# Krabbens/edge-diffusion-tts

Hardware: AMD Instinct MI355X
Metric: mel-frames/sec (whole node), 4-step DDIM, hidden=160 L=4, B=256 T=512 (higher is better)
Workload: dtype f32

## Files before the change

### edge-diffusion-tts_amd/csrc/edtts_device.h

```cpp
#pragma once
#include <hip/hip_runtime.h>
#include <stdint.h>
#include <type_traits>

#if !defined(EDTTS_EXPERIMENTS) &&                                                                                                  \
    (defined(EDTTS_STAMPS) || defined(EDTTS_STAMP_HEAD) || defined(EDTTS_STAMP_THREAD) || defined(EDTTS_WAVELOG) ||                 \
     defined(EDTTS_DS_STAMPS) || defined(EDTTS_FAST_BUILD))
#error "diagnostic and build switches are scratch-only: add -DEDTTS_EXPERIMENTS"
#endif
#if defined(EDTTS_W2) || defined(EDTTS_KV2) || defined(EDTTS_SPLITLOAD) || defined(EDTTS_SPLIT_ON) || defined(EDTTS_HANDOVER) ||    \
    defined(EDTTS_H_DMA) || defined(EDTTS_TAIL_RING2) || defined(EDTTS_DS_BURST) || defined(EDTTS_PIN_MASK) ||                      \
    defined(EDTTS_WMAX) || defined(EDTTS_RB) || defined(EDTTS_ABLATE_QKVSTORES) || defined(EDTTS_ABLATE_KVLOADS) ||                 \
    defined(EDTTS_DS_ABL) || defined(EDTTS_DIAG) || defined(EDTTS16_HP) || defined(EDTTS16_KVDEPTH) ||                              \
    defined(EDTTS16_MFMA_SUM) || defined(EDTTS16_EVEN_STEPS) || defined(EDTTS16_QLDS) || defined(EDTTS16_IMG) ||                    \
    defined(EDTTS16_W1) || defined(EDTTS16_NF) || defined(EDTTS16_ABLATE_BARRIER) || defined(EDTTS16_ABLATE_DMA) ||                 \
    defined(EDTTS16_PHASES)
#error "this switch is retired, see DESIGN.md: its variant was decided and the code removed (last present in c6f336d)"
#endif

constexpr int kPinMask = 0x4;
#define EDTTS_PIN_ACC(x) asm volatile("" : "+a"(x))
typedef float f4 __attribute__((ext_vector_type(4)));
typedef float f2 __attribute__((ext_vector_type(2)));

#define EDTTS_MFMA(a, b, c) __builtin_amdgcn_mfma_f32_16x16x4f32((a), (b), (c), 0, 0, 0)
#define EDTTS_DEV __device__ __forceinline__

#ifdef EDTTS_STAMPS
#define STAMP_SEL_HEAD(sel) ((sel) & 0xff)
#define STAMPX(p, i, sel) do { if ((p) && (int)blockIdx.x == ((sel) >> 16) && (int)threadIdx.x == 64 * (((sel) >> 8) & 0xff)) (p)[i] = __builtin_amdgcn_s_memtime(); } while (0)
#else
#define STAMPX(p, i, sel) do { } while (0)
#endif

namespace edtts {

constexpr int kCtxWaves = 4;

template <int H_, int HEADS_, int MEL_, int NF_ = 2>
struct Cfg {
  static constexpr int H = H_, HEADS = HEADS_, MEL = MEL_, NF = NF_;
  static constexpr int WF = 16 * NF;
  static constexpr int QT = NF >= 2 ? 2 : 1;
  static constexpr int NHALF = NF / QT;
  static constexpr int DH = H / HEADS;
  static constexpr int DFULL = DH / 16;
  static constexpr int DREM = DH % 16;
  static constexpr int DT = (DH + 15) / 16;
  static constexpr int DHP = DT * 16;
  static constexpr int HT = H / 16;
  static constexpr int MT = MEL / 16;
  static constexpr int R = H / 2, RT = R / 16;
  static constexpr int VR = (HEADS - 1) * DH + DHP;
  static constexpr int WMAX = 2;
  static constexpr int WAVES0 = (HT * NF * 4 <= 160) ? 4 : 2;
  static constexpr int WAVES = NF == 1 ? 1 : (WAVES0 < WMAX ? WAVES0 : WMAX);
// ... 572 lines not shown
#ifdef EDTTS_STAMPS
        if (hd == STAMP_SEL_HEAD(stamp_sel)) STAMPX(stamps, sidx++, stamp_sel);
#endif
      };
      const int cd = q.cdiag;
      auto chunk_of = [&](int st) { return st >= nchunk ? nchunk - 1 : (st == 0 ? cd : (st <= cd ? st - 1 : st)); };
      constexpr bool HANDOVER = NHALF == 1;
      const bool more = HANDOVER && hd + hstep < C::HEADS;
      auto req_head = [&](int st) { return (more && st == nchunk - 1) ? hd + hstep : hd; };
      auto req_chunk = [&](int st) { return (more && st == nchunk - 1) ? cd : chunk_of(st + 1); };
      step(No{}, cd, req_chunk(0), KA, VA, req_head(0));
      for (int st = 1; st < nchunk; ++st) step(Yes{}, chunk_of(st), req_chunk(st), KA, VA, req_head(st));
#pragma unroll
      for (int ft = 0; ft < QT; ++ft) {
        const float lt = group_sum(hsum(lvec[ft]));
        const float inv = lt > 0.f ? 1.0f / lt : 0.f;
#pragma unroll
        for (int dt = 0; dt < DT; ++dt) O[dt][QT * hf + ft] *= inv;
      }
    }
#ifdef EDTTS_STAMPS
    if (hd == STAMP_SEL_HEAD(stamp_sel)) STAMPX(stamps, sidx++, stamp_sel);
#endif
    if (hd + hstep < C::HEADS) {
      if constexpr (NHALF == 1) {
        load_q(hd + hstep, 0);
        __builtin_amdgcn_sched_barrier(0);
      } else {
        prefetch(geo[0], hd + hstep, 0);
      }
    }
    if constexpr (OMODE == O_LDS) {
      char* ob = obuf + hd * C::OHEAD_BYTES;
#pragma unroll
      for (int dt = 0; dt < DT; ++dt)
#pragma unroll
        for (int ft = 0; ft < NF; ++ft) {
          if (DREM && dt == DT - 1) reinterpret_cast<f2*>(ob + DFULL * NF * 1024 + ft * 512)[lane] = f2{O[dt][ft][0], O[dt][ft][1]};
          else reinterpret_cast<f4*>(ob + (dt * NF + ft) * 1024)[lane] = O[dt][ft];
        }
    } else {
#pragma unroll
      for (int dt = 0; dt < DT; ++dt) {
        if (DREM && dt == DT - 1) ktile_phase<C::HT, WStream<C>::RN_, NF, 2>(ring, O[dt], h);
        else ktile_phase<C::HT>(ring, O[dt], h);
      }
    }
#ifdef EDTTS_STAMPS
    if (hd == STAMP_SEL_HEAD(stamp_sel)) STAMPX(stamps, sidx++, stamp_sel);
#endif
  }
}

EDTTS_DEV void ddim_elem(float x, float e, float s1m, float sab, float sabp, float cdir, float& x0, float& xp) {
#pragma clang fp contract(off)
  float t1 = s1m * e;
  float t2 = x - t1;
  float v = div_rn(t2, sab);
  v = fminf(fmaxf(v, -3.0f), 3.0f);
  x0 = v;
  float t3 = sabp * v;
  float t4 = cdir * e;
  xp = t3 + t4;
}
struct DdimCoef {
  float s1m, sab, sabp, cdir, sigma;
};
EDTTS_DEV DdimCoef ddim_coef(float ab, float abp, float eta) {
#pragma clang fp contract(off)
  DdimCoef c;
  c.s1m = sqrt_rn(1.0f - ab);
  c.sab = sqrt_rn(ab);
  float r1 = div_rn(1.0f - abp, 1.0f - ab);
  float r2 = 1.0f - div_rn(ab, abp);
  float pr = r1 * r2;
  c.sigma = eta * sqrt_rn(pr);
  float s2 = c.sigma * c.sigma;
  float in = 1.0f - abp;
  in = in - s2;
  c.cdir = sqrt_rn(in);
  c.sabp = sqrt_rn(abp);
  return c;
}
EDTTS_DEV float add_mul_rn(float p, float s, float n) {
#pragma clang fp contract(off)
  float t = s * n;
  return p + t;
}

struct DdpmCoef {
  float coef1, coef2, sd;
};
EDTTS_DEV DdpmCoef ddpm_coef(float al, float ab, float be, float var, bool nonzero) {
#pragma clang fp contract(off)
  DdpmCoef c;
  c.coef1 = div_rn(1.0f, sqrt_rn(al));
  float om = 1.0f - ab;
  c.coef2 = div_rn(be, sqrt_rn(om));
  c.sd = (nonzero ? 1.0f : 0.0f) * sqrt_rn(var);
  return c;
}
EDTTS_DEV float ddpm_elem(float x, float e, float n, DdpmCoef c) {
#pragma clang fp contract(off)
  float t1 = c.coef2 * e;
  float t2 = x - t1;
  float mean = c.coef1 * t2;
  float t3 = c.sd * n;
  return mean + t3;
}

struct LmsCoef {
  int mode;
  float p0, p1, c0, c1, rinv, cB, cC;
};
EDTTS_DEV void lms_elem(float x, float out, float h_new, float h_old, const LmsCoef& k, float& x0, float& xn) {
#pragma clang fp contract(off)
// ... 139 lines not shown
```

### edge-diffusion-tts_amd/csrc/edtts_generic.h

```cpp
namespace edtts_gen {

enum { EPI_BIAS = 0, EPI_PE = 1, EPI_RESID = 2, EPI_SWIGLU = 3 };

struct GemmArgs {
  const float* X;
  const float* W;
  const float* bias;
  float* Y;
  const float* pe;
  int M, N, K, ldx, ldy, T;
  int vec_x, vec_w, vec_y;
  DropArgs dr;
};
constexpr int kGBM = 64, kGBN = 64, kGBK = 16, kGLd = kGBK + 1;

template <int EPI, bool DROP = false>
__global__ __launch_bounds__(256) void k_gen_gemm(GemmArgs a) {
  __shared__ float xs[kGBM][kGLd];
  __shared__ float ws[kGBN][kGLd];
  const int tid = threadIdx.x, lane = tid & 63, w = tid >> 6, fq = lane & 15, g = lane >> 4;
  const int m0 = blockIdx.x * kGBM;
  const int n0 = blockIdx.y * (EPI == EPI_SWIGLU ? kGBN / 2 : kGBN);
  const int lr = tid >> 2, lk = 4 * (tid & 3);
  int wrow;
// ... 280 lines not shown
                                                   int H, int n_tok, unsigned* err, const int64_t* s_len) {
  const size_t n = (size_t)rows * H;
  for (size_t i = (size_t)blockIdx.x * blockDim.x + threadIdx.x; i < n; i += (size_t)gridDim.x * blockDim.x) {
    const size_t row = i / H;
    const int c = (int)(i - row * H);
    long tk = (s_len && (int)(row % S) >= utt_len_lane(s_len, (int)(row / S), S)) ? 0 : (long)sem_idx[row];
    if (tk < 0 || tk >= n_tok) {
      if (c == 0) atomicOr(err, (unsigned)EDTTS_IDX_SEM);
      tk = tk < 0 ? 0 : n_tok - 1;
    }
    ctx[i] = tok[(size_t)tk * H + c] + cpe[(size_t)(row % S) * H + c];
  }
}

template <int TAIL>
EDTTS_DEV void tail_elem(const KArgs& a, size_t idx, float e) {
  if (TAIL == TAIL_LMS) {
    const float hn = a.lms.mode >= 2 ? a.h_new[idx] : 0.f, ho = a.lms.mode >= 3 ? a.h_old[idx] : 0.f;
    float v0, vn;
    lms_elem(a.x[idx], e, hn, ho, a.lms, v0, vn);
    a.x0_hist[idx] = v0;
    if (a.x0_all) a.x0_all[idx] = v0;
    a.x_prev[idx] = vn;
  } else if (TAIL == TAIL_VLMS) {
    const float v = a.v_uncond ? cfg_combine(e, a.v_uncond[idx], a.vp.cfg) : e;
    const float hn = a.lms.mode >= 2 ? a.h_new[idx] : 0.f, ho = a.lms.mode >= 3 ? a.h_old[idx] : 0.f;
    float v0, vn;
    lms_elem(a.x[idx], v, hn, ho, a.lms, v0, vn);
    a.x0_hist[idx] = v0;
    if (a.x0_all) a.x0_all[idx] = v0;
    if (a.known != nullptr) {
      const size_t row = (size_t)a.T * a.inj_mel, b = idx / row, r = idx - b * row, per = (size_t)a.inj_frames * a.inj_mel;
      if (r < per) {
        const size_t ki = b * per + r;
        vn = a.known[ki];
        if (a.p_coef2 != 0.f) {
          const float nz = a.noise ? a.noise[ki]
                                   : (a.seeds ? philox_normal4(a.seeds[b], a.step, r >> 2)[(int)(r & 3)] : philox_normal4(a.seed, a.step, ki >> 2)[(int)(ki & 3)]);
          vn = qsample_elem(vn, a.p_coef1, nz, a.p_coef2);
        }
      }
    }
    a.x_prev[idx] = vn;
  } else if (TAIL == TAIL_VPRED) {
    const float v = a.v_uncond ? cfg_combine(e, a.v_uncond[idx], a.vp.cfg) : e;
    a.x_prev[idx] = vpred_elem(a.x[idx], v, a.vp);
  } else if (TAIL == TAIL_DDPM) {
    const unsigned long long ge = a.philox_base + idx;
    const float nz = a.noise ? a.noise[idx] : philox_normal4(a.seed, a.step, ge >> 2)[(int)(ge & 3)];
    const DdpmCoef cf{a.p_coef1, a.p_coef2, a.p_sd};
    a.x_prev[idx] = ddpm_elem(a.x[idx], e, nz, cf);
  } else {
    float v0, vp;
    ddim_elem(a.x[idx], e, a.c_s1m, a.c_sab, a.c_sabp, a.c_dir, v0, vp);
    a.x0[idx] = v0;
    a.x_prev[idx] = vp;
  }
}
template <int TAIL>
EDTTS_DEV void tail_zero_elem(const KArgs& a, size_t idx) {
  if (TAIL == TAIL_LMS || TAIL == TAIL_VLMS) {
    a.x0_hist[idx] = 0.f;
    if (a.x0_all) a.x0_all[idx] = 0.f;
  } else if (TAIL == TAIL_DDIM) {
    a.x0[idx] = 0.f;
  }
  a.x_prev[idx] = 0.f;
}
EDTTS_DEV bool past_len(const int64_t* t_len, bool dbl, size_t idx, int T, int MEL) {
  if (t_len == nullptr) return false;
  const size_t row = idx / MEL;
  return (int)(row % T) >= utt_len_lane(t_len, (int)(row / T), T, dbl);
}
template <int TAIL>
__global__ __launch_bounds__(256) void k_gen_tail(KArgs a, const float* eps, size_t n, int vec, int MEL) {
  const size_t stride = (size_t)gridDim.x * blockDim.x;
  if (vec) {
    for (size_t i = (size_t)blockIdx.x * blockDim.x + threadIdx.x; i < n / 4; i += stride) {
      if constexpr (TAIL == TAIL_VLMS) {
        const size_t row = 4 * i / MEL;
        const int f = (int)(row % a.T);
        const int Tb = a.t_len ? utt_len_of(a.t_len[row / a.T], a.T, a.t_dbl) : a.T;
        tail_store<TAIL>(a, f, Tb, 4 * i, ldg4(eps + 4 * i));
        continue;
      }
      if (past_len(a.t_len, a.t_dbl, 4 * i, a.T, MEL)) tail_zero<TAIL>(a, 4 * i);
      else tail_apply<TAIL>(a, 4 * i, ldg4(eps + 4 * i));
    }
  } else {
    for (size_t i = (size_t)blockIdx.x * blockDim.x + threadIdx.x; i < n; i += stride) {
      if (past_len(a.t_len, a.t_dbl, i, a.T, MEL)) tail_zero_elem<TAIL>(a, i);
      else tail_elem<TAIL>(a, i, eps[i]);
    }
  }
}
__global__ __launch_bounds__(256) void k_gen_zero_past(float* y, const int64_t* t_len, int dbl, size_t n, int T, int MEL) {
  for (size_t i = (size_t)blockIdx.x * blockDim.x + threadIdx.x; i < n; i += (size_t)gridDim.x * blockDim.x)
    if (past_len(t_len, dbl, i, T, MEL)) y[i] = 0.f;
}

}

enum { DROP_ATTN = 0, DROP_CROSS = 1, DROP_ACT = 2, DROP_DOWN = 3 };
struct DropState {
  unsigned k0, k1, thr;
  float scale;
  DropArgs site(int layer, int site_id) const { return DropArgs{k0, k1, 0x30000u + 4u * (unsigned)layer + (unsigned)site_id, thr, scale}; }
};

struct FwdLayerBufs {
  float *crp, *crn, *kv;
  float *qkv, *att1, *lse1;
  float *qc, *att2, *lse2;
  float* act;
  float *h0, *h1, *h2;
};
struct FwdBufs {
  float* ctx;
// ... 201 lines not shown
```

### edge-diffusion-tts_amd/csrc/edtts_kernels.hip

```cpp
#include <hip/hip_runtime.h>
#include <math.h>
#include <stdarg.h>
#include <stdlib.h>
#include <stdio.h>
#include <string.h>
#include <atomic>
#include <initializer_list>
#include <mutex>
#include <vector>

#include "../../include/edtts.h"
#include "edtts_device.h"

using namespace edtts;

static thread_local char g_err[512] = "";
static int fail(int code, const char* fmt, ...) __attribute__((format(printf, 2, 3)));
static int fail(int code, const char* fmt, ...) {
  va_list ap;
  va_start(ap, fmt);
  vsnprintf(g_err, sizeof(g_err), fmt, ap);
  va_end(ap);
  return code;
}
// ... 374 lines not shown
    sidx = a.use_host ? (long)a.step_host[row] : (long)a.step_idx[row];
    if (sidx < 0 || sidx >= a.n_step) {
      if (tid == 0) atomicOr(a.err, (unsigned)EDTTS_IDX_STEP);
      sidx = sidx < 0 ? 0 : a.n_step - 1;
    }
  }
  for (int n = tid; n < H; n += blockDim.x) {
    float acc = a.t3b[n];
#pragma unroll 8
    for (int k = 0; k < H; ++k) acc = fmaf(u[k], a.t3T[(size_t)k * H + n], acc);
    if (sidx >= 0) acc += a.step[(size_t)sidx * H + n];
    a.tcond[(size_t)row * H + n] = acc;
  }
}
__global__ __launch_bounds__(256) void k_cond_ada(CondArgs a) {
  extern __shared__ float sm[];
  const int row = blockIdx.x, lw = blockIdx.y, l = lw >> 1, which = lw & 1, H = a.H;
  for (int k = threadIdx.x; k < H; k += blockDim.x) sm[k] = a.tcond[(size_t)row * H + k];
  __syncthreads();
  const float* WT = a.blob + (which ? a.ada3T[l] : a.ada1T[l]);
  const float* bb = a.blob + (which ? a.ada3b[l] : a.ada1b[l]);
  float* out = a.cond + (((size_t)row * a.L + l) * 2 + which) * 2 * H;
  for (int n = blockIdx.z * blockDim.x + threadIdx.x; n < 2 * H; n += gridDim.z * blockDim.x) {
    float acc = bb[n];
#pragma unroll 8
    for (int k = 0; k < H; ++k) acc = fmaf(sm[k], WT[(size_t)k * 2 * H + n], acc);
    out[n] = n < H ? 1.0f + acc : acc;
  }
}

struct KArgs {
  int B, T, Tp, S, Sp, window, max_pos, max_cpos, n_tok, SD, L;
  const float* x;
  float* h;
  const float *q, *k, *vT;
  float *q_out, *k_out, *vT_out;
  float *kc, *vcT;
  const float* known;
  const unsigned long long* seeds;
  int inj_frames, inj_mel;
  const int64_t* sem_idx;
  const float* sem_feat;
  const float* cond;
  int cond_bstride;
  int layer;
  int ffn_tiles;
  int diag_skip;
  unsigned long long* stamps;
  const float *tok, *semp, *semp_b, *cpe, *inp, *inp_b, *pe;
  const float *n1w, *proj_b, *n2w, *n3w, *up_b, *down_b, *fnw, *fnb, *outp_b;
  const float* stream;
  float *eps, *x_prev, *x0;
  float c_s1m, c_sab, c_sabp, c_dir;
  float p_coef1, p_coef2, p_sd;
  const float* noise;
  unsigned long long seed;
  unsigned long long philox_base;
  unsigned step;
  LmsCoef lms;
  VpredCoef vp;
  const float* v_uncond;
  const float *h_new, *h_old;
  float *x0_hist, *x0_all;
  const int64_t *t_len, *s_len;
  int t_dbl;
};

EDTTS_DEV int utt_len_of(int64_t v, int full, bool dbl) {
  const int hi = dbl ? full >> 1 : full;
  const int n = v < 1 ? 1 : (v > hi ? hi : (int)v);
  return dbl ? 2 * n : n;
}
EDTTS_DEV int utt_len(const int64_t* len, int b, int full, bool dbl = false) {
  if (len == nullptr) return full;
  return utt_len_of(len[__builtin_amdgcn_readfirstlane(b)], full, dbl);
}
EDTTS_DEV int utt_len_lane(const int64_t* len, int b, int full, bool dbl = false) {
  return len == nullptr ? full : utt_len_of(len[b], full, dbl);
}
EDTTS_DEV int live_end(int n) { return (n + 31) & ~31; }

EDTTS_DEV int remap_block(int bid, int nblk) {
  const int q = nblk >> 3, r = nblk & 7, xcd = bid & 7, idx = bid >> 3;
  const int base = xcd < r ? xcd * (q + 1) : r * (q + 1) + (xcd - r) * q;
  return base + idx;
}

struct TileId {
  int b, m0;
  bool valid;
};
EDTTS_DEV TileId wave_tile(int B, int Tp, int waves_per_block, int wave_frames) {
  const int wave = __builtin_amdgcn_readfirstlane(threadIdx.x >> 6);
  const int tpu = Tp / wave_frames;
  int w = remap_block(blockIdx.x, gridDim.x) * waves_per_block + wave;
  TileId t;
  t.valid = w < B * tpu;
  w = t.valid ? w : B * tpu - 1;
  t.b = w / tpu;
  t.m0 = (w - t.b * tpu) * wave_frames;
  return t;
}

template <class C>
EDTTS_DEV void qkv_tail(WStream<C>& ring0, const f4 (&hn)[C::HT][C::NF], const KArgs& a, int b, int m0, int lane) {
  constexpr int NF = C::NF;
// ... 59 lines not shown
  }
  f4 h[C::HT][NF];
#pragma unroll
  for (int nt = 0; nt < C::HT; ++nt) {
    const f4 bias = ldg4(a.inp_b + 16 * nt + 4 * g);
#pragma unroll
    for (int ft = 0; ft < NF; ++ft) h[nt][ft] = bias;
  }
  {
    constexpr int N = C::HT * C::MT;
    static_assert(N % WStream<C>::RN_ == 0 && C::HT % 2 == 0, "in_proj must be a whole number of ring turns");
#pragma unroll
    for (int nt = 0; nt < C::HT; nt += 2)
#pragma unroll
      for (int kt = 0; kt < C::MT; ++kt) {
        const int i = nt * C::MT + 2 * kt;
        const f4& fa = ring.at(i);
        const f4& fb = ring.at(i + 1);
#pragma unroll
        for (int r = 0; r < 4; ++r) {
#pragma unroll
          for (int ft = 0; ft < NF; ++ft) h[nt][ft] = EDTTS_MFMA(fa[r], xin[kt][ft][r], h[nt][ft]);
#pragma unroll
          for (int ft = 0; ft < NF; ++ft) h[nt + 1][ft] = EDTTS_MFMA(fb[r], xin[kt][ft][r], h[nt + 1][ft]);
        }
        ring.template refill_after<N>(i);
        ring.template refill_after<N>(i + 1);
      }
    ring.advance(N);
  }
#pragma unroll
  for (int ft = 0; ft < NF; ++ft) {
    int f = m0 + 16 * ft + fq;
    f = f < a.max_pos ? f : a.max_pos - 1;
#pragma unroll
    for (int nt = 0; nt < C::HT; ++nt) h[nt][ft] += ldg4(a.pe + (size_t)f * C::H + 16 * nt + 4 * g);
  }
  {
    float* hp = a.h + ((size_t)b * a.Tp + m0 + fq) * C::H + 4 * g;
#pragma unroll
    for (int nt = 0; nt < C::HT; ++nt)
#pragma unroll
      for (int ft = 0; ft < NF; ++ft) stg4(hp + 16 * nt + (size_t)ft * 16 * C::H, h[nt][ft]);
  }
  f4 hn[C::HT][NF];
  const float* mod = a.cond + (size_t)b * a.cond_bstride;
  rms_norm_tile<C::HT, NF>(h, a.n1w, mod, g, hn);
  qkv_tail<C>(ring, hn, a, b, m0, lane);
}

enum { TAIL_QKV = 0, TAIL_EPS = 1, TAIL_DDIM = 2, TAIL_DDPM = 3, TAIL_LMS = 4, TAIL_VPRED = 5, TAIL_VLMS = 6 };

template <int TAIL>
EDTTS_DEV void tail_apply(const KArgs& a, size_t idx, f4 ev, bool blend = false) {
  if (TAIL == TAIL_EPS) {
    stg4(a.eps + idx, ev);
  } else if (TAIL == TAIL_LMS) {
    const f4 xv = ldg4(a.x + idx);
    f4 hn = splat(0.f), ho = splat(0.f);
    if (a.lms.mode >= 2) hn = ldg4(a.h_new + idx);
    if (a.lms.mode >= 3) ho = ldg4(a.h_old + idx);
    f4 x0, xn;
#pragma unroll
    for (int r = 0; r < 4; ++r) {
      float v0, vn;
      lms_elem(xv[r], ev[r], hn[r], ho[r], a.lms, v0, vn);
      x0[r] = v0;
      xn[r] = vn;
    }
    stg4(a.x0_hist + idx, x0);
    if (a.x0_all) stg4(a.x0_all + idx, x0);
    stg4(a.x_prev + idx, xn);
  } else if (TAIL == TAIL_VLMS) {
    const bool guided = a.v_uncond != nullptr;
    const f4 xv = ldg4(a.x + idx);
    const f4 vu = ldg4((guided ? a.v_uncond : a.x) + idx);
    f4 hn = splat(0.f), ho = splat(0.f);
    if (a.lms.mode >= 2) hn = ldg4(a.h_new + idx);
    if (a.lms.mode >= 3) ho = ldg4(a.h_old + idx);
    f4 x0, xn;
#pragma unroll
    for (int r = 0; r < 4; ++r) {
      const float v = guided ? cfg_combine(ev[r], vu[r], a.vp.cfg) : ev[r];
      float v0, vn;
      lms_elem(xv[r], v, hn[r], ho[r], a.lms, v0, vn);
      x0[r] = v0;
      xn[r] = vn;
    }
    stg4(a.x0_hist + idx, x0);
    if (a.x0_all) stg4(a.x0_all + idx, x0);
    if (!blend) stg4(a.x_prev + idx, xn);
  } else if (TAIL == TAIL_VPRED) {
    const bool guided = a.v_uncond != nullptr;
    const f4 xv = ldg4(a.x + idx);
    const f4 vu = ldg4((guided ? a.v_uncond : a.x) + idx);
    f4 v, xn;
#pragma unroll
    for (int r = 0; r < 4; ++r) v[r] = guided ? cfg_combine(ev[r], vu[r], a.vp.cfg) : ev[r];
#pragma unroll
    for (int r = 0; r < 4; ++r) xn[r] = vpred_elem(xv[r], v[r], a.vp);
    stg4(a.x_prev + idx, xn);
  } else if (TAIL == TAIL_DDPM) {
    const f4 xv = ldg4(a.x + idx);
    const f4 nz = a.noise ? ldg4(a.noise + idx) : philox_normal4(a.seed, a.step, (a.philox_base + idx) >> 2);
    const DdpmCoef cf{a.p_coef1, a.p_coef2, a.p_sd};
    f4 xp;
#pragma unroll
    for (int r = 0; r < 4; ++r) xp[r] = ddpm_elem(xv[r], ev[r], nz[r], cf);
    stg4(a.x_prev + idx, xp);
  } else {
    const f4 xv = ldg4(a.x + idx);
    f4 x0, xp;
#pragma unroll
    for (int r = 0; r < 4; ++r) {
      float v0, vp;
      ddim_elem(xv[r], ev[r], a.c_s1m, a.c_sab, a.c_sabp, a.c_dir, v0, vp);
      x0[r] = v0;
      xp[r] = vp;
    }
    stg4(a.x0 + idx, x0);
    stg4(a.x_prev + idx, xp);
  }
}
template <int TAIL>
EDTTS_DEV void tail_zero(const KArgs& a, size_t idx) {
  const f4 z = splat(0.f);
  if (TAIL == TAIL_EPS) {
    stg4(a.eps + idx, z);
  } else if (TAIL == TAIL_LMS || TAIL == TAIL_VLMS) {
    stg4(a.x0_hist + idx, z);
    if (a.x0_all) stg4(a.x0_all + idx, z);
    stg4(a.x_prev + idx, z);
  } else if (TAIL == TAIL_DDIM) {
    stg4(a.x0 + idx, z);
    stg4(a.x_prev + idx, z);
  } else {
    stg4(a.x_prev + idx, z);
  }
}
EDTTS_DEV void vlms_blend(const KArgs& a, size_t idx) {
  const size_t row = (size_t)a.T * a.inj_mel, b = idx / row, r = idx - b * row;
  const size_t ki = b * ((size_t)a.inj_frames * a.inj_mel) + r;
  const f4 kv = ldg4(a.known + ki);
  f4 o = kv;
  if (a.p_coef2 != 0.f) {
    const unsigned long long sd = a.seeds ? a.seeds[b] : a.seed;
    const f4 nz = a.noise ? ldg4(a.noise + ki) : philox_normal4(sd, a.step, (a.seeds ? r : ki) >> 2);
#pragma unroll
    for (int e = 0; e < 4; ++e) o[e] = qsample_elem(kv[e], a.p_coef1, nz[e], a.p_coef2);
  }
  stg4(a.x_prev + idx, o);
}
template <int TAIL>
EDTTS_DEV void tail_store(const KArgs& a, int f, int Tb, size_t idx, f4 ev) {
  if constexpr (TAIL == TAIL_VLMS) {
    const bool blend = a.known != nullptr && f < Tb && f < a.inj_frames;
    if (f < Tb) tail_apply<TAIL>(a, idx, ev, blend);
    else tail_zero<TAIL>(a, idx);
    if (blend) vlms_blend(a, idx);
  } else {
    if (f < Tb) tail_apply<TAIL>(a, idx, ev);
    else tail_zero<TAIL>(a, idx);
  }
}

struct QGlobal {
  __amdgpu_buffer_rsrc_t rs;
  unsigned v4, v2;
  int H;
  EDTTS_DEV QGlobal(const float* row_m0, int H_, int fq, int g) : rs(make_rsrc(row_m0)), v4((unsigned)(fq * H_ + 4 * g) * 4u), v2((unsigned)(fq * H_ + 2 * g) * 4u), H(H_) {}
  EDTTS_DEV f4 q4(int ft, int col) const { return bufld4(rs, v4, (unsigned)(ft * 16 * H + col) * 4u); }
  EDTTS_DEV f2 q2(int ft, int col) const { return bufld2(rs, v2, (unsigned)(ft * 16 * H + col) * 4u); }
};
struct QLds {
  const float* b4;
  const float* b2;
  int ld;
  EDTTS_DEV QLds(const float* tile, int ld_, int fq, int g) : b4(tile + fq * ld_ + 4 * g), b2(tile + fq * ld_ + 2 * g), ld(ld_) {}
  EDTTS_DEV f4 q4(int ft, int col) const { return *reinterpret_cast<const f4*>(b4 + ft * 16 * ld + col); }
  EDTTS_DEV f2 q2(int ft, int col) const { return *reinterpret_cast<const f2*>(b2 + ft * 16 * ld + col); }
};

template <class C, int TAIL>
EDTTS_DEV void layer_tile(const KArgs& a, float* smem, int wave, int lane, int b, int m0, int Tb, int Sb) {
  constexpr int NF = C::NF;
  const int fq = lane & 15, g = lane >> 4;
  f4* const stash = reinterpret_cast<f4*>(smem) + (size_t)wave * C::HT * NF * 64 + lane;
  constexpr int QLDS = C::H;
  float* qtile = smem + (size_t)C::WAVES * C::HT * NF * 256 + (size_t)wave * C::WF * QLDS;
  const size_t rowbase = (size_t)b * a.Tp + m0 + fq;

  STAMPX(a.stamps, 0, a.diag_skip);
  WStream<C> ring;
  ring.prime(a.stream, lane);

  f4 h[C::HT][NF];
  float* const hp = a.h + rowbase * C::H + 4 * g;
  auto park_h = [&]() {
#pragma unroll
    for (int nt = 0; nt < C::HT; ++nt)
#pragma unroll
      for (int ft = 0; ft < NF; ++ft) stash[(nt * NF + ft) * 64] = h[nt][ft];
  };
  auto add_parked_h = [&]() {
#pragma unroll
    for (int nt = 0; nt < C::HT; ++nt)
#pragma unroll
      for (int ft = 0; ft < NF; ++ft) h[nt][ft] += stash[(nt * NF + ft) * 64];
  };
  {
#pragma unroll
    for (int nt = 0; nt < C::HT; ++nt)
#pragma unroll
      for (int ft = 0; ft < NF; ++ft) h[nt][ft] = ldg4(hp + 16 * nt + (size_t)ft * 16 * C::H);
// ... 42 lines not shown
    zero_h();
    if constexpr (C::Q_IN_LDS) {
      QLds ql(qtile, QLDS, fq, g);
      attention_fused<C, false, O_FUSED>(ql, a.kc + (size_t)b * a.Sp * C::H, a.vcT + (size_t)b * C::VR * a.Sp, a.Sp, Sb, -1, m0, lane, ring, h,
                                         nullptr, []() {}, a.stamps ? a.stamps + 40 : nullptr, a.diag_skip);
    } else {
      QGlobal ql(a.q + ((size_t)b * a.Tp + m0) * C::H, C::H, fq, g);
      attention_fused<C, false, O_FUSED>(ql, a.kc + (size_t)b * a.Sp * C::H, a.vcT + (size_t)b * C::VR * a.Sp, a.Sp, Sb, -1, m0, lane, ring, h,
                                         nullptr, []() {});
    }
    add_parked_h();
    STAMPX(a.stamps, 3, a.diag_skip);
  }
  {
    f4 hn[C::HT][NF];
    const float* mod = a.cond + (size_t)b * a.cond_bstride + ((size_t)a.layer * 2 + 1) * 2 * C::H;
    rms_norm_tile<C::HT, NF>(h, a.n3w, mod, g, hn);
    park_h();
#pragma unroll
    for (int nt = 0; nt < C::HT; ++nt) {
      const f4 db = ldg4(a.down_b + 16 * nt + 4 * g);
#pragma unroll
      for (int ft = 0; ft < NF; ++ft) h[nt][ft] = db;
    }
    for (int j = 0; j < a.ffn_tiles; ++j) {
      const f4 vb = ldg4(a.up_b + 32 * j + 4 * g), gb = ldg4(a.up_b + 32 * j + 16 + 4 * g);
      f4 v[NF], gt[NF], act[NF];
#pragma unroll
      for (int ft = 0; ft < NF; ++ft) v[ft] = gt[ft] = splat(0.f);
      gemm_phase_pair<C::HT>(ring, hn, v, gt);
      __builtin_amdgcn_sched_barrier(0);
#pragma unroll
      for (int ft = 0; ft < NF; ++ft) act[ft] = swiglu_tile(v[ft], gt[ft], vb, gb);
      __builtin_amdgcn_sched_barrier(0);
      ktile_phase<C::HT>(ring, act, h);
    }
    add_parked_h();
    STAMPX(a.stamps, 4, a.diag_skip);
  }
  if (TAIL == TAIL_QKV) {
    {
      float* hp = a.h + rowbase * C::H + 4 * g;
#pragma unroll
      for (int nt = 0; nt < C::HT; ++nt)
#pragma unroll
        for (int ft = 0; ft < NF; ++ft) stg4(hp + 16 * nt + (size_t)ft * 16 * C::H, h[nt][ft]);
    }
    const float* mod = a.cond + (size_t)b * a.cond_bstride + ((size_t)(a.layer + 1) * 2) * 2 * C::H;
    rms_norm_tile<C::HT, NF>(h, a.n1w, mod, g, h);
    qkv_tail<C>(ring, h, a, b, m0, lane);
  } else {
    f4 hn[C::HT][NF];
    layer_norm_tile<C::HT, NF>(h, a.fnw, a.fnb, g, hn);
#pragma unroll
    for (int nt = 0; nt < C::MT; ++nt) {
      const f4 ob = ldg4(a.outp_b + 16 * nt + 4 * g);
      f4 e[NF];
#pragma unroll
      for (int ft = 0; ft < NF; ++ft) e[ft] = splat(0.f);
      gemm_phase<C::HT>(ring, hn, e);
#pragma unroll
      for (int ft = 0; ft < NF; ++ft) {
        const int f = m0 + 16 * ft + fq;
        if (f >= a.T) continue;
        const size_t idx = ((size_t)b * a.T + f) * C::MEL + 16 * nt + 4 * g;
        tail_store<TAIL>(a, f, Tb, idx, e[ft] + ob);
      }
    }
  }
  STAMPX(a.stamps, 5, a.diag_skip);
#ifdef EDTTS_STAMPS
  asm volatile("s_waitcnt vmcnt(0)" ::: "memory");
#endif
  STAMPX(a.stamps, 6, a.diag_skip);
}

template <class C, int TAIL>
EDTTS_DEV void tail_zero_tile(const KArgs& a, int b, int m0, int lane) {
  const int fq = lane & 15, g = lane >> 4;
#pragma unroll
  for (int ft = 0; ft < C::NF; ++ft) {
    const int f = m0 + 16 * ft + fq;
    if (f >= a.T) continue;
#pragma unroll
    for (int nt = 0; nt < C::MT; ++nt) tail_zero<TAIL>(a, ((size_t)b * a.T + f) * C::MEL + 16 * nt + 4 * g);
  }
}
template <class C, int TAIL>
__global__ __launch_bounds__(C::THREADS, 1) void k_layer(KArgs a) {
  extern __shared__ __attribute__((aligned(16))) float smem[];
  const int lane = threadIdx.x & 63;
  const int wave = __builtin_amdgcn_readfirstlane(threadIdx.x >> 6);
  const TileId tl = wave_tile(a.B, a.Tp, C::WAVES, C::WF);
  if (!tl.valid) return;
  const int Tb = utt_len(a.t_len, tl.b, a.T, a.t_dbl);
  if (tl.m0 >= live_end(Tb)) {
    if constexpr (TAIL != TAIL_QKV) tail_zero_tile<C, TAIL>(a, tl.b, tl.m0, lane);
    return;
  }
  const int Sb = utt_len(a.s_len, tl.b, a.S);
#ifdef EDTTS_WAVELOG
  const unsigned long long wl_r0 = __builtin_amdgcn_s_memrealtime(), wl_c0 = __builtin_amdgcn_s_memtime();
#endif
  layer_tile<C, TAIL>(a, smem, wave, lane, tl.b, tl.m0, Tb, Sb);
#ifdef EDTTS_WAVELOG
  if (a.stamps && lane == 0) {
    asm volatile("s_waitcnt vmcnt(0)" ::: "memory");
    unsigned long long* p = a.stamps + 6 * ((size_t)a.diag_skip + (size_t)tl.b * (a.Tp / C::WF) + tl.m0 / C::WF);
    p[0] = wl_r0; p[1] = wl_c0; p[2] = __builtin_amdgcn_s_memrealtime(); p[3] = __builtin_amdgcn_s_memtime();
    p[4] = __builtin_amdgcn_s_getreg((31 << 11) | 4);
    p[5] = __builtin_amdgcn_s_getreg((31 << 11) | 20);
  }
#endif
}

#include "edtts_coop.h"
#include "edtts_bf16.h"

struct CtxArgs {
// ... 1130 lines not shown
struct DdpmStepArgs {
  const float* noise;
  unsigned long long seed, base;
  unsigned step;
};
struct VpredStepArgs {
  VpredCoef k;
  const float* v_uncond;
};
struct LmsStepArgs {
  LmsCoef k;
  const float *h_new, *h_old;
  float *x0_hist, *x0_all;
};
struct BlendStepArgs {
  const float *known, *noise;
  int frames, mel;
  float c_known, c_noise;
  unsigned long long seed;
  const unsigned long long* seeds;
  unsigned step;
};
struct StepTail {
  int kind = TAIL_EPS;
  float* eps = nullptr;
  float* x_prev = nullptr;
  float* x0 = nullptr;
  const float* coef = nullptr;
  DdpmStepArgs ddpm{};
  LmsStepArgs lms{};
  VpredStepArgs vp{};
  BlendStepArgs blend{};
};
static void set_tail_args(const StepTail& t, KArgs* a) {
  if (t.kind == TAIL_EPS) {
    a->eps = t.eps;
    return;
  }
  a->x_prev = t.x_prev;
  if (t.kind == TAIL_LMS || t.kind == TAIL_VLMS) {
    a->lms = t.lms.k; a->h_new = t.lms.h_new; a->h_old = t.lms.h_old; a->x0_hist = t.lms.x0_hist; a->x0_all = t.lms.x0_all;
    if (t.kind == TAIL_LMS) return;
    a->vp = t.vp.k; a->v_uncond = t.vp.v_uncond;
    a->known = t.blend.known; a->noise = t.blend.noise; a->inj_frames = t.blend.frames; a->inj_mel = t.blend.mel;
    a->p_coef1 = t.blend.c_known; a->p_coef2 = t.blend.c_noise; a->seed = t.blend.seed; a->seeds = t.blend.seeds; a->step = t.blend.step;
  } else if (t.kind == TAIL_VPRED) {
    a->vp = t.vp.k; a->v_uncond = t.vp.v_uncond;
  } else if (t.kind == TAIL_DDPM) {
    a->p_coef1 = t.coef[0]; a->p_coef2 = t.coef[1]; a->p_sd = t.coef[2];
    a->noise = t.ddpm.noise; a->seed = t.ddpm.seed; a->philox_base = t.ddpm.base; a->step = t.ddpm.step;
  } else {
    a->x0 = t.x0;
    a->c_s1m = t.coef[0]; a->c_sab = t.coef[1]; a->c_sabp = t.coef[2]; a->c_dir = t.coef[3];
  }
}
template <class F>
static int with_tail(int kind, F&& f) {
  switch (kind) {
    case TAIL_QKV: return f(std::integral_constant<int, TAIL_QKV>{});
    case TAIL_EPS: return f(std::integral_constant<int, TAIL_EPS>{});
    case TAIL_LMS: return f(std::integral_constant<int, TAIL_LMS>{});
    case TAIL_DDPM: return f(std::integral_constant<int, TAIL_DDPM>{});
    case TAIL_VPRED: return f(std::integral_constant<int, TAIL_VPRED>{});
    case TAIL_VLMS: return f(std::integral_constant<int, TAIL_VLMS>{});
    default: return f(std::integral_constant<int, TAIL_DDIM>{});
  }
}
#define TRY_G(x) do { int rc_ = (x); if (rc_) return rc_; } while (0)
template <class F>
static int for_each_tail(F&& f) {
  for (int kind : {TAIL_QKV, TAIL_EPS, TAIL_DDIM, TAIL_DDPM, TAIL_LMS, TAIL_VPRED, TAIL_VLMS}) TRY_G(with_tail(kind, f));
  return EDTTS_OK;
}
struct Lens {
  const int64_t *t = nullptr, *s = nullptr;
  bool t_dbl = false;
  Lens at(int off) const { return Lens{t ? t + off : nullptr, s ? s + off : nullptr, t_dbl}; }
};
struct CallCtx {
  const Layout& lo;
  const float* blob;
  Workspace ws;
  float* wsb;
  int B, T, S, window;
  Lens ln;
  hipStream_t st;
};

#ifdef EDTTS_STAMPS
static unsigned long long* g_stamps_fwd = nullptr;
#endif
#ifdef EDTTS_WAVELOG
static unsigned long long* g_wavelog = nullptr;
static thread_local int g_wavelog_base = 0;
#endif

static CtxArgs ctx_args(const CallCtx& c, const int64_t* sem_idx, const float* sem_feat) {
  const Layout& lo = c.lo;
  CtxArgs a;
  memset(&a, 0, sizeof(a));
  a.B = c.B; a.S = c.S; a.Sp = c.ws.Sp; a.L = lo.L; a.SD = lo.SD; a.n_tok = lo.NTOK; a.max_cpos = lo.MAXCPOS;
  a.sem_idx = sem_idx; a.sem_feat = sem_feat; a.s_len = c.ln.s;
  a.tok = c.blob + lo.tok; a.semp = c.blob + lo.semp; a.semp_b = c.blob + lo.semp_b; a.cpe = c.blob + lo.cpe; a.blob = c.blob;
  for (int l = 0; l < lo.L; ++l) {
    a.kvd[l] = (unsigned)lo.layer[l].kvd; a.kvn[l] = (unsigned)lo.layer[l].kvn; a.kvu[l] = (unsigned)lo.layer[l].kvu;
  }
// ... 673 lines not shown
```

### edge-diffusion-tts_amd/csrc/edtts_samplers.h

```cpp

struct StepArgs {
  const float *alphas, *alpha_bar, *betas, *post_var;
  int n_table;
  const float *x, *eps, *noise;
  const int64_t *t, *t_prev;
  size_t n_per_batch;
  float eta;
  float *x_prev, *x0;
  int vec4;
};
static int step_vec4(size_t n_per_batch, std::initializer_list<const void*> ptrs) {
  uintptr_t m = 0;
  for (const void* p : ptrs) m |= (uintptr_t)p;
  return (n_per_batch & 3) == 0 && (m & 15) == 0;
}
EDTTS_DEV long clamp_idx(long v, int n) { return v < 0 ? 0 : (v >= n ? n - 1 : v); }

__global__ __launch_bounds__(256) void k_ddim(StepArgs a) {
  const int b = blockIdx.y;
  const float ab = a.alpha_bar[clamp_idx((long)a.t[b], a.n_table)];
  const long tp = (long)a.t_prev[b];
  const float abp = tp >= 0 ? a.alpha_bar[clamp_idx(tp, a.n_table)] : 1.0f;
  const DdimCoef cf = ddim_coef(ab, abp, a.eta);
  const float s1m = cf.s1m, sab = cf.sab, sabp = cf.sabp, cdir = cf.cdir, sigma = cf.sigma;
  const size_t base = (size_t)b * a.n_per_batch;
  const size_t n4 = a.vec4 ? a.n_per_batch >> 2 : 0;
  for (size_t i = (size_t)blockIdx.x * blockDim.x + threadIdx.x; i < n4; i += (size_t)gridDim.x * blockDim.x) {
    const size_t o = base + 4 * i;
    const f4 xv = ldg4(a.x + o), e = ldg4(a.eps + o);
    f4 nz = splat(0.f);
    if (a.noise) nz = ldg4(a.noise + o);
    f4 x0, xp;
#pragma unroll
    for (int r = 0; r < 4; ++r) {
      float v, p;
      ddim_elem(xv[r], e[r], s1m, sab, sabp, cdir, v, p);
      if (a.noise) p = add_mul_rn(p, sigma, nz[r]);
      x0[r] = v;
      xp[r] = p;
    }
    stg4(a.x0 + o, x0);
    stg4(a.x_prev + o, xp);
  }
  for (size_t i = (n4 << 2) + (size_t)blockIdx.x * blockDim.x + threadIdx.x; i < a.n_per_batch; i += (size_t)gridDim.x * blockDim.x) {
    const size_t o = base + i;
    float v, p;
    ddim_elem(a.x[o], a.eps[o], s1m, sab, sabp, cdir, v, p);
    if (a.noise) p = add_mul_rn(p, sigma, a.noise[o]);
    a.x0[o] = v;
    a.x_prev[o] = p;
  }
}

__global__ __launch_bounds__(256) void k_ddpm(StepArgs a) {
  const int b = blockIdx.y;
  const long tt = clamp_idx((long)a.t[b], a.n_table);
  const float al = a.alphas[tt], ab = a.alpha_bar[tt], be = a.betas[tt];
  const DdpmCoef cf = ddpm_coef(al, ab, be, a.post_var[tt], (long)a.t[b] > 0);
  const size_t base = (size_t)b * a.n_per_batch;
  const size_t n4 = a.vec4 ? a.n_per_batch >> 2 : 0;
  for (size_t i = (size_t)blockIdx.x * blockDim.x + threadIdx.x; i < n4; i += (size_t)gridDim.x * blockDim.x) {
    const size_t o = base + 4 * i;
    const f4 xv = ldg4(a.x + o), e = ldg4(a.eps + o), nz = ldg4(a.noise + o);
    f4 xp;
#pragma unroll
    for (int r = 0; r < 4; ++r) xp[r] = ddpm_elem(xv[r], e[r], nz[r], cf);
    stg4(a.x_prev + o, xp);
  }
  for (size_t i = (n4 << 2) + (size_t)blockIdx.x * blockDim.x + threadIdx.x; i < a.n_per_batch; i += (size_t)gridDim.x * blockDim.x) {
    const size_t o = base + i;
    a.x_prev[o] = ddpm_elem(a.x[o], a.eps[o], a.noise[o], cf);
  }
}

extern "C" {

__global__ __launch_bounds__(256) void k_inpaint_inject(float* x, const float* known, const float* noise, int B, int T, int ov, int MEL,
                                                        float c_known, float c_noise, unsigned long long seed, unsigned step,
                                                        const unsigned long long* seeds, const int64_t* t_len) {
  const size_t per = (size_t)ov * MEL / 4, n4 = (size_t)B * per;
  for (size_t i = (size_t)blockIdx.x * blockDim.x + threadIdx.x; i < n4; i += (size_t)gridDim.x * blockDim.x) {
    const size_t b = i / per, r = i - b * per;
    const int Tb = t_len ? utt_len_of(t_len[b], T, false) : T;
    const size_t live = Tb < ov ? (size_t)Tb * MEL : 4 * per;
    if (4 * r >= live) continue;
    const f4 kv = ldg4(known + 4 * i);
    f4 o = kv;
    if (c_noise != 0.f) {
      const f4 nz = noise ? ldg4(noise + 4 * i) : (seeds ? philox_normal4(seeds[b], step, r) : philox_normal4(seed, step, i));
#pragma unroll
      for (int e = 0; e < 4; ++e) o[e] = qsample_elem(kv[e], c_known, nz[e], c_noise);
    }
    if (4 * r + 4 <= live) {
      stg4(x + (b * T) * MEL + 4 * r, o);
    } else {
#pragma unroll
      for (int e = 0; e < 4; ++e)
        if (4 * r + e < live) x[(b * T) * MEL + 4 * r + e] = o[e];
    }
  }
// ... 144 lines not shown
        eps_tail.eps = a.v_uncond;
        TRY_G(LN::forward(cu, a.x, wsb + ws.cond + i * row, 0, eps_tail));
        tail.vp.v_uncond = a.v_uncond;
      }
      TRY_G(LN::forward(c, a.x, wsb + ws.cond + i * row, 0, tail));
    }
    if (a.known_mel) TRY_G(inject_after());
  });
  return EDTTS_OK;
}

static void launch_inject(const InpaintArgs& a, int mel, float c_known, float c_noise, int step) {
  const size_t per_k = (size_t)a.B * a.overlap_len * mel;
  const bool vec = ((size_t)a.overlap_len * mel) % 4 == 0 && ((size_t)a.T * mel) % 4 == 0;
  const size_t bx = (per_k / (vec ? 4 : 1) + 255) / 256;
  hipLaunchKernelGGL(vec ? k_inpaint_inject : k_inpaint_inject1, dim3(bx > 2048 ? 2048u : (unsigned)bx), dim3(256), 0, (hipStream_t)a.stream, a.x, a.known_mel,
                     a.noise_k ? a.noise_k + (size_t)step * per_k : nullptr, a.B, a.T, a.overlap_len, mel, c_known, c_noise,
                     (unsigned long long)a.seed, kStreamInpaintStep + (unsigned)step, reinterpret_cast<const unsigned long long*>(a.seeds),
                     a.t_len);
}

static unsigned step_blocks(const StepArgs& a) {
  const size_t bx = ((a.vec4 ? a.n_per_batch / 4 : a.n_per_batch) + 255) / 256;
  return bx > 2048 ? 2048u : (bx < 1 ? 1u : (unsigned)bx);
}

extern "C" {

int edtts_generate(const EdttsDims* dims, const void* packed, void* workspace, int B, int S, const int64_t* sem_idx,
                   const float* x_T, int num_steps, const int64_t* timesteps_host, const float* coef_host, float* x_work,
                   float* x0_out, void* stream) {
  return edtts_generate_len(dims, packed, workspace, B, S, sem_idx, nullptr, x_T, num_steps, timesteps_host, coef_host, x_work, x0_out,
                            stream);
}

int edtts_generate_len(const EdttsDims* dims, const void* packed, void* workspace, int B, int S, const int64_t* sem_idx,
                       const int64_t* s_len, const float* x_T, int num_steps, const int64_t* timesteps_host, const float* coef_host,
                       float* x_work, float* x0_out, void* stream) {
  const SettingsScope settings;
  Layout lo;
  TRY_G(make_layout(dims, &lo));
  if (!packed || !workspace || !sem_idx || !x_T || !timesteps_host || !coef_host || !x_work || !x0_out)
    return fail(EDTTS_ERR_ARG, "NULL pointer argument");
  if (num_steps < 1 || num_steps > lo.NSTEP)
    return fail(EDTTS_ERR_ARG, "num_steps=%d outside [1,%d] (step_emb rows; the reference raises IndexError)", num_steps, lo.NSTEP);
  const int T = 2 * S;
  TRY_G(check_shapes(lo, B, T, S));
  SamplerInputs in;
  in.t_host = timesteps_host; in.sem_idx = sem_idx;
  in.ln = Lens{s_len, s_len, true};
  in.x_T = x_T; in.x = x_work;
  return run_sampler(dims, lo, packed, workspace, B, T, S, num_steps, in, stream, [&](int i, int, size_t o) {
    StepTail tail;
    tail.kind = TAIL_DDIM; tail.x_prev = x_work + o; tail.x0 = x0_out + o; tail.coef = coef_host + 4 * i;
    return tail;
  });
}

int edtts_sample_multistep(const EdttsDims* dims, const void* packed, void* workspace, int B, int T, int S, const int64_t* sem_idx,
                           const float* sem_features, const float* x_T, int num_steps, const int64_t* timesteps_host,
                           const float* coef_host, float* hist, float* x0_all, float* x_out, void* stream) {
  return edtts_sample_multistep_len(dims, packed, workspace, B, T, S, sem_idx, sem_features, nullptr, nullptr, x_T, num_steps,
                                    timesteps_host, coef_host, hist, x0_all, x_out, stream);
}

int edtts_sample_multistep_len(const EdttsDims* dims, const void* packed, void* workspace, int B, int T, int S, const int64_t* sem_idx,
                               const float* sem_features, const int64_t* t_len, const int64_t* s_len, const float* x_T, int num_steps,
                               const int64_t* timesteps_host, const float* coef_host, float* hist, float* x0_all, float* x_out,
                               void* stream) {
  const SettingsScope settings;
  Layout lo;
  TRY_G(make_layout(dims, &lo));
  if (!sem_idx && !sem_features) return fail(EDTTS_ERR_ARG, "Either sem_idx or sem_features must be provided");
  if (!packed || !workspace || !x_T || !timesteps_host || !coef_host || !hist || !x_out) return fail(EDTTS_ERR_ARG, "NULL pointer argument");
  if (num_steps < 1 || num_steps > lo.NSTEP)
    return fail(EDTTS_ERR_ARG, "num_steps=%d outside [1,%d] (step_emb rows; the reference raises IndexError)", num_steps, lo.NSTEP);
  TRY_G(check_shapes(lo, B, T, S));
  TRY_G(check_lms_modes(coef_host, num_steps));
  SamplerInputs in;
  in.t_host = timesteps_host; in.sem_idx = sem_idx; in.sem_features = sem_features;
  in.ln = Lens{t_len, s_len};
  in.x_T = x_T; in.x = x_out;
  const size_t per = (size_t)B * T * lo.MEL;
  return run_sampler(dims, lo, packed, workspace, B, T, S, num_steps, in, stream, [&](int i, int, size_t o) {
    StepTail tail;
    tail.kind = TAIL_LMS; tail.x_prev = x_out + o;
    tail.lms = lms_step_args(coef_host + 8 * i, hist, x0_all, per, i, o);
    return tail;
  });
}

int edtts_sample_ddpm(const EdttsDims* dims, const void* packed, void* workspace, int B, int S, const int64_t* sem_idx,
                      const float* x_T, int num_steps, const int64_t* t_all, const float* coef_host, const float* noise_all,
                      uint64_t seed, int64_t batch_offset, float* x_out, void* stream) {
  return edtts_sample_ddpm_len(dims, packed, workspace, B, S, sem_idx, nullptr, x_T, num_steps, t_all, coef_host, noise_all, seed,
                               batch_offset, x_out, stream);
}

int edtts_sample_ddpm_len(const EdttsDims* dims, const void* packed, void* workspace, int B, int S, const int64_t* sem_idx,
                          const int64_t* s_len, const float* x_T, int num_steps, const int64_t* t_all, const float* coef_host,
                          const float* noise_all, uint64_t seed, int64_t batch_offset, float* x_out, void* stream) {
  const SettingsScope settings;
  Layout lo;
  TRY_G(make_layout(dims, &lo));
  if (!packed || !workspace || !sem_idx || !x_T || !t_all || !coef_host || !x_out) return fail(EDTTS_ERR_ARG, "NULL pointer argument");
  if (num_steps < 1) return fail(EDTTS_ERR_ARG, "num_steps=%d < 1", num_steps);
  if (batch_offset < 0) return fail(EDTTS_ERR_ARG, "batch_offset=%lld < 0", (long long)batch_offset);
// ... 157 lines not shown
```

Baseline: 8.719 million.

## Replace DDIM divide with verified reciprocal, skip intermediate x0 stores, prefetch x

Replaces the correctly rounded division in the DDIM update with a multiply by a host-verified reciprocal plus an FMA correction step. It falls back to div_rn when the reciprocal check fails or operands are out of range. x0 is now written only on the final step of generate, which removes a full-tensor store on every earlier step. The fused tail also loads x ahead of the output projection loop so the load latency can overlap with compute. This adds range checks per element and a second code path that must stay bit-exact.

Result: no change. 8.740 million, median of 3 (+0.2%).

```diff
diff --git a/edge-diffusion-tts_amd/csrc/edtts_device.h b/edge-diffusion-tts_amd/csrc/edtts_device.h
--- a/edge-diffusion-tts_amd/csrc/edtts_device.h
+++ b/edge-diffusion-tts_amd/csrc/edtts_device.h
@@ -2,6 +2,7 @@
 #include <hip/hip_runtime.h>
 #include <stdint.h>
 #include <type_traits>
+#include "edtts_exact_div.h"
 
 #if !defined(EDTTS_EXPERIMENTS) &&                                                                                                  \
     (defined(EDTTS_STAMPS) || defined(EDTTS_STAMP_HEAD) || defined(EDTTS_STAMP_THREAD) || defined(EDTTS_WAVELOG) ||                 \
@@ -680,16 +681,44 @@
   }
 }
 
-EDTTS_DEV void ddim_elem(float x, float e, float s1m, float sab, float sabp, float cdir, float& x0, float& xp) {
+EDTTS_DEV void ddim_elem(float x, float e, float s1m, float sab, float rsab, float sabp, float cdir, float& x0, float& xp) {
 #pragma clang fp contract(off)
   float t1 = s1m * e;
   float t2 = x - t1;
-  float v = div_rn(t2, sab);
+  float v;
+  if (__builtin_expect(rsab != 0.f && exact_div_ok(t2), 1)) v = exact_div(t2, sab, rsab);
+  else v = div_rn(t2, sab);
   v = fminf(fmaxf(v, -3.0f), 3.0f);
   x0 = v;
   float t3 = sabp * v;
   float t4 = cdir * e;
   xp = t3 + t4;
+}
+EDTTS_DEV void ddim_quad(f4 x, f4 e, float s1m, float sab, float rsab, float sabp, float cdir, f4& x0, f4& xp) {
+#pragma clang fp contract(off)
+  f4 t2, v;
+#pragma unroll
+  for (int r = 0; r < 4; ++r) {
+    float t1 = s1m * e[r];
+    t2[r] = x[r] - t1;
+  }
+  const float hi = fmaxf(fmaxf(fabsf(t2[0]), fabsf(t2[1])), fmaxf(fabsf(t2[2]), fabsf(t2[3])));
+  const float lo = fminf(fminf(fabsf(t2[0]), fabsf(t2[1])), fminf(fabsf(t2[2]), fabsf(t2[3])));
+  if (__builtin_expect(rsab != 0.f && lo >= kExactDivMinA && hi <= kExactDivMaxA, 1)) {
+#pragma unroll
+    for (int r = 0; r < 4; ++r) v[r] = exact_div(t2[r], sab, rsab);
+  } else {
+#pragma unroll
+    for (int r = 0; r < 4; ++r) v[r] = div_rn(t2[r], sab);
+  }
+#pragma unroll
+  for (int r = 0; r < 4; ++r) {
+    float c = fminf(fmaxf(v[r], -3.0f), 3.0f);
+    x0[r] = c;
+    float t3 = sabp * c;
+    float t4 = cdir * e[r];
+    xp[r] = t3 + t4;
+  }
 }
 struct DdimCoef {
   float s1m, sab, sabp, cdir, sigma;
diff --git a/edge-diffusion-tts_amd/csrc/edtts_exact_div.h b/edge-diffusion-tts_amd/csrc/edtts_exact_div.h
--- /dev/null
+++ b/edge-diffusion-tts_amd/csrc/edtts_exact_div.h
@@ -0,0 +1,52 @@
+#pragma once
+#include <math.h>
+#include <stdint.h>
+
+#if defined(__HIPCC__) || defined(__CUDACC__)
+#define EDTTS_HD __host__ __device__ inline
+#else
+#define EDTTS_HD inline
+#endif
+
+namespace edtts {
+
+constexpr float kExactDivMinA = 0x1p-40f, kExactDivMaxA = 0x1p64f;
+constexpr float kExactDivMinB = 0x1p-20f, kExactDivMaxB = 0x1p20f;
+
+EDTTS_HD uint32_t exact_div_bits(float v) {
+  uint32_t u;
+  __builtin_memcpy(&u, &v, 4);
+  return u;
+}
+EDTTS_HD float exact_div_from_bits(uint32_t u) {
+  float v;
+  __builtin_memcpy(&v, &u, 4);
+  return v;
+}
+
+EDTTS_HD bool exact_div_check(float b, float y) {
+  if (!(b >= kExactDivMinB && b <= kExactDivMaxB)) return false;
+  if ((exact_div_bits(b) & 0x7fffffu) == 0x7fffffu) return false;
+  if (!(y > 0.f && y <= 2.0f / kExactDivMinB)) return false;
+  const double db = (double)b;
+  const double e0 = fabs(1.0 - db * (double)y);
+  const double em = fabs(1.0 - db * (double)exact_div_from_bits(exact_div_bits(y) - 1u));
+  const double ep = fabs(1.0 - db * (double)exact_div_from_bits(exact_div_bits(y) + 1u));
+  return e0 < em && e0 < ep;
+}
+EDTTS_HD float exact_div_recip(float b) {
+  const float y = (float)(1.0 / (double)b);
+  return exact_div_check(b, y) ? y : 0.f;
+}
+EDTTS_HD bool exact_div_ok(float a) {
+  const float m = fabsf(a);
+  return m >= kExactDivMinA && m <= kExactDivMaxA;
+}
+EDTTS_HD float exact_div(float a, float b, float y) {
+#pragma clang fp contract(off)
+  const float q = a * y;
+  const float r = __builtin_fmaf(-b, q, a);
+  return __builtin_fmaf(r, y, q);
+}
+
+}
diff --git a/edge-diffusion-tts_amd/csrc/edtts_generic.h b/edge-diffusion-tts_amd/csrc/edtts_generic.h
--- a/edge-diffusion-tts_amd/csrc/edtts_generic.h
+++ b/edge-diffusion-tts_amd/csrc/edtts_generic.h
@@ -356,8 +356,8 @@
     a.x_prev[idx] = ddpm_elem(a.x[idx], e, nz, cf);
   } else {
     float v0, vp;
-    ddim_elem(a.x[idx], e, a.c_s1m, a.c_sab, a.c_sabp, a.c_dir, v0, vp);
-    a.x0[idx] = v0;
+    ddim_elem(a.x[idx], e, a.c_s1m, a.c_sab, a.c_rsab, a.c_sabp, a.c_dir, v0, vp);
+    if (a.x0) a.x0[idx] = v0;
     a.x_prev[idx] = vp;
   }
 }
@@ -367,7 +367,7 @@
     a.x0_hist[idx] = 0.f;
     if (a.x0_all) a.x0_all[idx] = 0.f;
   } else if (TAIL == TAIL_DDIM) {
-    a.x0[idx] = 0.f;
+    if (a.x0) a.x0[idx] = 0.f;
   }
   a.x_prev[idx] = 0.f;
 }
diff --git a/edge-diffusion-tts_amd/csrc/edtts_kernels.hip b/edge-diffusion-tts_amd/csrc/edtts_kernels.hip
--- a/edge-diffusion-tts_amd/csrc/edtts_kernels.hip
+++ b/edge-diffusion-tts_amd/csrc/edtts_kernels.hip
@@ -450,6 +450,7 @@
   const float* stream;
   float *eps, *x_prev, *x0;
   float c_s1m, c_sab, c_sabp, c_dir;
+  float c_rsab;
   float p_coef1, p_coef2, p_sd;
   const float* noise;
   unsigned long long seed;
@@ -615,7 +616,7 @@
 enum { TAIL_QKV = 0, TAIL_EPS = 1, TAIL_DDIM = 2, TAIL_DDPM = 3, TAIL_LMS = 4, TAIL_VPRED = 5, TAIL_VLMS = 6 };
 
 template <int TAIL>
-EDTTS_DEV void tail_apply(const KArgs& a, size_t idx, f4 ev, bool blend = false) {
+EDTTS_DEV void tail_apply(const KArgs& a, size_t idx, f4 ev, bool blend = false, const f4* x_pre = nullptr) {
   if (TAIL == TAIL_EPS) {
     stg4(a.eps + idx, ev);
   } else if (TAIL == TAIL_LMS) {
@@ -672,16 +673,10 @@
     for (int r = 0; r < 4; ++r) xp[r] = ddpm_elem(xv[r], ev[r], nz[r], cf);
     stg4(a.x_prev + idx, xp);
   } else {
-    const f4 xv = ldg4(a.x + idx);
+    const f4 xv = x_pre ? *x_pre : ldg4(a.x + idx);
     f4 x0, xp;
-#pragma unroll
-    for (int r = 0; r < 4; ++r) {
-      float v0, vp;
-      ddim_elem(xv[r], ev[r], a.c_s1m, a.c_sab, a.c_sabp, a.c_dir, v0, vp);
-      x0[r] = v0;
-      xp[r] = vp;
-    }
-    stg4(a.x0 + idx, x0);
+    ddim_quad(xv, ev, a.c_s1m, a.c_sab, a.c_rsab, a.c_sabp, a.c_dir, x0, xp);
+    if (a.x0) stg4(a.x0 + idx, x0);
     stg4(a.x_prev + idx, xp);
   }
 }
@@ -695,7 +690,7 @@
     if (a.x0_all) stg4(a.x0_all + idx, z);
     stg4(a.x_prev + idx, z);
   } else if (TAIL == TAIL_DDIM) {
-    stg4(a.x0 + idx, z);
+    if (a.x0) stg4(a.x0 + idx, z);
     stg4(a.x_prev + idx, z);
   } else {
     stg4(a.x_prev + idx, z);
@@ -715,14 +710,14 @@
   stg4(a.x_prev + idx, o);
 }
 template <int TAIL>
-EDTTS_DEV void tail_store(const KArgs& a, int f, int Tb, size_t idx, f4 ev) {
+EDTTS_DEV void tail_store(const KArgs& a, int f, int Tb, size_t idx, f4 ev, const f4* x_pre = nullptr) {
   if constexpr (TAIL == TAIL_VLMS) {
     const bool blend = a.known != nullptr && f < Tb && f < a.inj_frames;
     if (f < Tb) tail_apply<TAIL>(a, idx, ev, blend);
     else tail_zero<TAIL>(a, idx);
     if (blend) vlms_blend(a, idx);
   } else {
-    if (f < Tb) tail_apply<TAIL>(a, idx, ev);
+    if (f < Tb) tail_apply<TAIL>(a, idx, ev, false, x_pre);
     else tail_zero<TAIL>(a, idx);
   }
 }
@@ -871,6 +866,17 @@
   } else {
     f4 hn[C::HT][NF];
     layer_norm_tile<C::HT, NF>(h, a.fnw, a.fnb, g, hn);
+    constexpr bool X_PRE = TAIL == TAIL_DDIM;
+    f4 xq[X_PRE ? C::MT : 1][NF];
+    if constexpr (X_PRE) {
+#pragma unroll
+      for (int nt = 0; nt < C::MT; ++nt)
+#pragma unroll
+        for (int ft = 0; ft < NF; ++ft) {
+          const int f = m0 + 16 * ft + fq;
+          xq[nt][ft] = f < a.T ? ldg4(a.x + ((size_t)b * a.T + f) * C::MEL + 16 * nt + 4 * g) : splat(0.f);
+        }
+    }
 #pragma unroll
     for (int nt = 0; nt < C::MT; ++nt) {
       const f4 ob = ldg4(a.outp_b + 16 * nt + 4 * g);
@@ -883,7 +889,7 @@
         const int f = m0 + 16 * ft + fq;
         if (f >= a.T) continue;
         const size_t idx = ((size_t)b * a.T + f) * C::MEL + 16 * nt + 4 * g;
-        tail_store<TAIL>(a, f, Tb, idx, e[ft] + ob);
+        tail_store<TAIL>(a, f, Tb, idx, e[ft] + ob, X_PRE ? &xq[nt][ft] : nullptr);
       }
     }
   }
@@ -2120,6 +2126,7 @@
   } else {
     a->x0 = t.x0;
     a->c_s1m = t.coef[0]; a->c_sab = t.coef[1]; a->c_sabp = t.coef[2]; a->c_dir = t.coef[3];
+    a->c_rsab = exact_div_recip(a->c_sab);
   }
 }
 template <class F>
diff --git a/edge-diffusion-tts_amd/csrc/edtts_samplers.h b/edge-diffusion-tts_amd/csrc/edtts_samplers.h
--- a/edge-diffusion-tts_amd/csrc/edtts_samplers.h
+++ b/edge-diffusion-tts_amd/csrc/edtts_samplers.h
@@ -23,6 +23,7 @@
   const float abp = tp >= 0 ? a.alpha_bar[clamp_idx(tp, a.n_table)] : 1.0f;
   const DdimCoef cf = ddim_coef(ab, abp, a.eta);
   const float s1m = cf.s1m, sab = cf.sab, sabp = cf.sabp, cdir = cf.cdir, sigma = cf.sigma;
+  const float rsab = exact_div_recip(sab);
   const size_t base = (size_t)b * a.n_per_batch;
   const size_t n4 = a.vec4 ? a.n_per_batch >> 2 : 0;
   for (size_t i = (size_t)blockIdx.x * blockDim.x + threadIdx.x; i < n4; i += (size_t)gridDim.x * blockDim.x) {
@@ -31,13 +32,10 @@
     f4 nz = splat(0.f);
     if (a.noise) nz = ldg4(a.noise + o);
     f4 x0, xp;
+    ddim_quad(xv, e, s1m, sab, rsab, sabp, cdir, x0, xp);
+    if (a.noise) {
 #pragma unroll
-    for (int r = 0; r < 4; ++r) {
-      float v, p;
-      ddim_elem(xv[r], e[r], s1m, sab, sabp, cdir, v, p);
-      if (a.noise) p = add_mul_rn(p, sigma, nz[r]);
-      x0[r] = v;
-      xp[r] = p;
+      for (int r = 0; r < 4; ++r) xp[r] = add_mul_rn(xp[r], sigma, nz[r]);
     }
     stg4(a.x0 + o, x0);
     stg4(a.x_prev + o, xp);
@@ -45,7 +43,7 @@
   for (size_t i = (n4 << 2) + (size_t)blockIdx.x * blockDim.x + threadIdx.x; i < a.n_per_batch; i += (size_t)gridDim.x * blockDim.x) {
     const size_t o = base + i;
     float v, p;
-    ddim_elem(a.x[o], a.eps[o], s1m, sab, sabp, cdir, v, p);
+    ddim_elem(a.x[o], a.eps[o], s1m, sab, rsab, sabp, cdir, v, p);
     if (a.noise) p = add_mul_rn(p, sigma, a.noise[o]);
     a.x0[o] = v;
     a.x_prev[o] = p;
@@ -296,7 +294,8 @@
   in.x_T = x_T; in.x = x_work;
   return run_sampler(dims, lo, packed, workspace, B, T, S, num_steps, in, stream, [&](int i, int, size_t o) {
     StepTail tail;
-    tail.kind = TAIL_DDIM; tail.x_prev = x_work + o; tail.x0 = x0_out + o; tail.coef = coef_host + 4 * i;
+    tail.kind = TAIL_DDIM; tail.x_prev = x_work + o; tail.coef = coef_host + 4 * i;
+    tail.x0 = i + 1 == num_steps ? x0_out + o : nullptr;
     return tail;
   });
 }
```
